# dattalab-6-cam/multicam-calibration

Hardware: AMD Instinct MI355X
Metric: LM iterations/sec (6 cams x 10k frames x 54 pts per GPU shard; + ms/Jacobian-eval) (higher is better)
Workload: dtype f64

## Files before the change

### multicam-calibration_amd/csrc/mcba_solve.hip

```cpp
#include <stdlib.h>
#include <algorithm>
#include "mcba_kernels.h"
#include "mcba_lm.h"
#include "mcba_math.h"
#include "mcba_backsub.h"

namespace mcba {

typedef double solve_d4 __attribute__((ext_vector_type(4)));

__device__ __forceinline__ double lane_bcast(double v, int lane) {
  union { double d; int i[2]; } a, b;
  a.d = v;
  b.i[0] = __builtin_amdgcn_readlane(a.i[0], lane);
  b.i[1] = __builtin_amdgcn_readlane(a.i[1], lane);
  return b.d;
}

__device__ __forceinline__ void wave_lds_sync() {
  __builtin_amdgcn_fence(__ATOMIC_RELEASE, "wavefront");
  __builtin_amdgcn_wave_barrier();
  __builtin_amdgcn_fence(__ATOMIC_ACQUIRE, "wavefront");
}

__device__ __forceinline__ double rsqrt_cubic(double a) {
  double y = __builtin_amdgcn_rsq(a);
  double e = fma(-a * y, y, 1.0);
  double q = e * fma(0.375, e, 0.5);
  return fma(y, q, y);
}

template <int NTHREADS>
__device__ __forceinline__ void block_reduce4(double (&v)[4], bool take_max, double* s_red) {
  const int wave = threadIdx.x >> 6, lane = threadIdx.x & 63;
#pragma unroll
  for (int off = 32; off >= 1; off >>= 1) {
#pragma unroll
    for (int c = 0; c < 4; ++c) {
      double o = __shfl_xor(v[c], off, 64);
      v[c] = take_max ? fmax(v[c], o) : v[c] + o;
    }
  }
  __syncthreads();
  if (lane == 0) {
#pragma unroll
    for (int c = 0; c < 4; ++c) s_red[c * 16 + wave] = v[c];
  }
  __syncthreads();
#pragma unroll
  for (int c = 0; c < 4; ++c) {
    double r = s_red[c * 16];
    for (int w = 1; w < NTHREADS / 64; ++w) r = take_max ? fmax(r, s_red[c * 16 + w]) : r + s_red[c * 16 + w];
    v[c] = r;
  }
}

__device__ __forceinline__ void post_state(const SolveArgs& a, const double* st, bool write_back, bool stepped = false) {
  const int tid = threadIdx.x;
  if (tid < MCBA_LMS - 1) {
    const double v = st[tid];
    if (write_back) a.lms[tid] = v;
    if (a.host_state) a.host_state[tid] = v;
  }
  if (!a.host_state && !a.flag) return;
  __threadfence_system();
  __syncthreads();
  if (tid == 0) {
    if (a.host_state) *reinterpret_cast<volatile double*>(a.host_state + MCBA_LMS - 1) = a.seq;
    if (a.flag) __hip_atomic_store(a.flag, 4.0 * a.seq + (stepped ? 2.0 : 3.0), __ATOMIC_RELEASE, __HIP_MEMORY_SCOPE_AGENT);
  }
}

#define STAMP(k) do { } while (0)

#ifndef MCBA_SOLVE_LOOKAHEAD
#define MCBA_SOLVE_LOOKAHEAD 1
#endif
__host__ __device__ inline bool solve_lookahead(int npad) { return MCBA_SOLVE_LOOKAHEAD && npad <= 96; }

#ifndef MCBA_RL_NB
#define MCBA_RL_NB 4
#endif
__device__ __forceinline__ void rl_lds_barrier() { asm volatile("s_waitcnt lgkmcnt(0)\n\ts_barrier" ::: "memory"); }
__device__ __forceinline__ size_t rl_tile(int I, int J) { return ((size_t)(I * (I + 1) / 2 + J)) << 8; }
typedef double solve_d2 __attribute__((ext_vector_type(2)));
__device__ __forceinline__ solve_d4 rl_tile_load(const double* t, int lane) {
  const solve_d2 lo = *reinterpret_cast<const solve_d2*>(t + 2 * lane), hi = *reinterpret_cast<const solve_d2*>(t + 128 + 2 * lane);
  return solve_d4{lo[0], lo[1], hi[0], hi[1]};
}
__device__ __forceinline__ void rl_tile_store(double* t, int lane, const solve_d4 v) {
  *reinterpret_cast<solve_d2*>(t + 2 * lane) = solve_d2{v[0], v[1]};
  *reinterpret_cast<solve_d2*>(t + 128 + 2 * lane) = solve_d2{v[2], v[3]};
}
__device__ __forceinline__ int rl_pi(int lane) { return ((lane & 3) << 2) | ((lane >> 2) & 3) | (lane & 48); }

__device__ __forceinline__ solve_d4 rl_system_load(const double* __restrict__ S0, int n, int I, int J, int lane) {
  const int row = 16 * I + (lane & 15), c0 = 16 * J + 4 * (lane >> 4);
  const bool in = row <= n && c0 < n;
  return *reinterpret_cast<const solve_d4*>(S0 + (in ? (size_t)row * n + c0 : 0));
}
__device__ __forceinline__ solve_d4 rl_system_fixup(solve_d4 v, const double* damp, const unsigned char* fixed, int n, int I, int J, int lane) {
  const int row = 16 * I + (lane & 15), c0 = 16 * J + 4 * (lane >> 4);
  const bool in = row <= n && c0 < n;
#pragma unroll
  for (int r = 0; r < 4; ++r) {
    const int c = c0 + r;
    double x = in ? v[r] : ((row == c) ? 1.0 : 0.0);
    if (in && row == c) x += damp[row];
    v[r] = x;
  }
  if (fixed) {
#pragma unroll
    for (int r = 0; r < 4; ++r) {
      const int c = c0 + r;
      const bool fr = row < n && fixed[min(row, n - 1)] != 0, fc = c < n && fixed[min(c, n - 1)] != 0;
      if (fr || fc) v[r] = (row == c) ? 1.0 : 0.0;
    }
  }
  return v;
}
__device__ __forceinline__ solve_d4 rl_tile_from_system(const double* __restrict__ S0, const double* damp, const unsigned char* fixed, int n, int I, int J, int lane) {
  return rl_system_fixup(rl_system_load(S0, n, I, J, lane), damp, fixed, n, I, J, lane);
}

__device__ __forceinline__ solve_d4 rl_update(solve_d4 c, const solve_d4 pj, const solve_d4 pi) {
#pragma unroll
  for (int s = 0; s < 4; ++s) c = __builtin_amdgcn_mfma_f64_16x16x4f64(-pj[s], pi[s], c, 0, 0, 0);
  return c;
}

__device__ __forceinline__ void rl_unflatten(int t, int& Ir, int& Jr) {
  Ir = (int)((sqrt(8.0 * t + 1.0) - 1.0) * 0.5);
  while ((Ir + 1) * (Ir + 2) / 2 <= t) ++Ir;
  while (Ir * (Ir + 1) / 2 > t) --Ir;
  Jr = t - Ir * (Ir + 1) / 2;
}

constexpr int kRlMaxStagers = 16;
__host__ __device__ inline int rl_stagers(int npad) { const int nblk = npad >> 4, moff = (nblk - 1) * (nblk - 2) / 2; return min(kRlMaxStagers, max(1, moff / 8)); }
__device__ __forceinline__ double* rl_stage_flags(const SolveArgs& a, int nblk) { return a.work + 2 * rl_tile(nblk, 0) + 256 * 8; }
__device__ __forceinline__ unsigned long long* rl_stage_claims(const SolveArgs& a, int nblk) { return reinterpret_cast<unsigned long long*>(rl_stage_flags(a, nblk) + kRlMaxStagers); }
__device__ __forceinline__ unsigned long long rl_stage_tag(const SolveArgs& a) { return (unsigned long long)fabs(a.stage_tag); }
struct RlNoGate { __device__ __forceinline__ bool operator()() const { return true; } };
template <class Gate = RlNoGate>
__device__ __forceinline__ void rl_stage_offdiag(const SolveArgs& a, int part, int nparts, int lane, int wave, Gate gate = Gate()) {
  const int n = a.n, nblk = a.npad >> 4, m = nblk - 2;
  if (m <= 0) { (void)gate(); return; }
  const int M = m * (m + 1) / 2;
  const int t_begin = (int)(((long long)M * part) / nparts), ntile = (int)(((long long)M * (part + 1)) / nparts) - t_begin;
  if (ntile <= 0) (void)gate();
  const double* __restrict__ S0 = a.red;
  double* T1 = a.work;
  int Ir, Jr;
  rl_unflatten(t_begin, Ir, Jr);
  for (int done = 0; done < ntile; done += 8) {
    solve_d4 v[8];
    double* dstp[8];
    int Is[8], Js[8];
#pragma unroll
    for (int j = 0; j < 8; ++j) {
      const bool ok = done + j < ntile;
      Is[j] = ok ? Ir + 2 : nblk - 1; Js[j] = ok ? Jr + 1 : nblk - 2;
      dstp[j] = ok ? T1 + rl_tile(Is[j], Js[j]) : a.work + 2 * rl_tile(nblk, 0) + 256 * wave;
      v[j] = rl_system_load(S0, n, Is[j], Js[j], lane);
      if (++Jr > Ir) { ++Ir; Jr = 0; }
    }
    if (done == 0 && !gate()) return;
#pragma unroll
    for (int j = 0; j < 8; ++j) rl_tile_store(dstp[j], lane, rl_system_fixup(v[j], nullptr, a.fixed, n, Is[j], Js[j], lane));
  }
}
__device__ __forceinline__ void rl_stager(const SolveArgs& a, int b, int ns) {
  if (a.stage_tag < 0.0) return;
  const int lane = threadIdx.x & 63, wave = __builtin_amdgcn_readfirstlane(threadIdx.x >> 6), nw = blockDim.x >> 6;
  extern __shared__ double smem[];
  volatile int* s_mine_p = reinterpret_cast<volatile int*>(smem);
#define s_mine (*s_mine_p)
  auto gate = [&]() -> bool {
    if (threadIdx.x == 0) {
      if (a.stage_tag != floor(a.stage_tag)) {
        const long long t0 = wall_clock64();
        while (wall_clock64() - t0 < 20000000LL) __builtin_amdgcn_s_sleep(64);
      }
      const unsigned long long tag2 = 2 * rl_stage_tag(a);
      const unsigned long long old = __hip_atomic_fetch_max(rl_stage_claims(a, a.npad >> 4) + b, tag2, __ATOMIC_RELAXED, __HIP_MEMORY_SCOPE_AGENT);
      s_mine = old < tag2 ? 1 : 0;
    }
    __syncthreads();
    return s_mine != 0;
  };
  rl_stage_offdiag(a, b * nw + wave, ns * nw, lane, wave & 7, gate);
  if (!s_mine) return;
#undef s_mine
  __threadfence();
  __syncthreads();
  if (threadIdx.x == 0) __hip_atomic_store(rl_stage_flags(a, a.npad >> 4) + b, a.stage_tag, __ATOMIC_RELEASE, __HIP_MEMORY_SCOPE_AGENT);
}

template <int NTHREADS>
__device__ __forceinline__ void solve_right_looking(const SolveArgs& a, const double* __restrict__ S0, const unsigned char* fixed, const double* damp, double* yv, double* dv, double* invd,
                                                    double* linv , double* Pop , double* dtile , double* znext , int* stage_miss , double* tstamp) {
  constexpr int NW = NTHREADS / 64, SL = 32 / NW;
  static_assert(NW == 8, "8 wavefronts: 256 VGPRs each");
  constexpr int NWK = NW - NW / 4;
  const int n = a.n, npad = a.npad, nblk = npad >> 4;
  const int tid = threadIdx.x, lane = tid & 63;
  const int wave = __builtin_amdgcn_readfirstlane(tid >> 6);
  const bool worker = (wave & 3) != 0;
  const int wk = wave - 1 - (wave >> 2);
  const int li = lane & 15, lg = lane >> 4, lpi = rl_pi(lane);
  double* T1 = a.work;
  double* T2 = a.work + rl_tile(nblk, 0);
  for (int j = tid; j < npad; j += NTHREADS) yv[j] = 0.0;
  solve_d4 Zp[SL];
#pragma unroll
  for (int sl = 0; sl < SL; ++sl) {
    const int I = wave + NW * sl;
    Zp[sl] = solve_d4{0.0, 0.0, 0.0, 0.0};
    if (I >= 1 && I < nblk) Zp[sl] = rl_tile_from_system(S0, damp, fixed, n, I, 0, lane);
    if (I == 1 && I < nblk) *reinterpret_cast<solve_d4*>(znext + 4 * lane) = Zp[sl];
  }
  if (wave == 0) {
    const solve_d4 v = rl_tile_from_system(S0, damp, fixed, n, 0, 0, lane);
#pragma unroll
    for (int r = 0; r < 4; ++r) dtile[li * 17 + 4 * lg + r] = v[r];
  }
  __syncthreads();
  for (int k = 0; k < nblk; ++k) {
    const int r0 = 16 * k;
    if (wave == 0) {
      double r[16];
#pragma unroll
      for (int c = 0; c < 16; ++c) r[c] = lane < 16 ? dtile[li * 17 + c] : ((lane < 32 && c == li) ? 1.0 : 0.0);
      double myinv = 1.0;
      const int jmax = r0 + 16 <= n ? 16 : n - r0;
#pragma unroll
      for (int j = 0; j < 16; ++j) {
        if (j < jmax) {
          double s0 = 0.0, s1 = 0.0;
#pragma unroll
          for (int qq = 0; qq < j; ++qq) {
            const double ljq = lane_bcast(r[qq], j);
            if (qq & 1) s1 = fma(r[qq], ljq, s1); else s0 = fma(r[qq], ljq, s0);
          }
          r[j] -= s0 + s1;
          const double pj = lane_bcast(r[j], j);
          const double inv = rsqrt_cubic(pj);
          r[j] *= inv;
          myinv = lane == j ? inv : myinv;
        }
      }
      if (lane < 16) {
        invd[r0 + lane] = myinv;
        if (r0 + lane == n) {
#pragma unroll
          for (int c = 0; c < 16; ++c) if (c < lane) yv[r0 + c] = r[c];
        }
      } else if (lane < 32) {
#pragma unroll
        for (int c = 0; c < 16; ++c) linv[(r0 + li) * 17 + c] = r[c];
      }
    } else {
    const int mleft = nblk - k - 1;
    const int nwk = k == 0 || mleft * (mleft + 1) / 2 >= 48 ? NWK + 1 : NWK;
    const int wq = worker ? wk : NWK;
    if (!worker && k > 0) {
      for (int I = k; I < nblk; ++I) {
        solve_d4 x;
#pragma unroll
        for (int r = 0; r < 4; ++r) x[r] = Pop[256 * I + 4 * ((4 * lg + r) + 16 * (li >> 2)) + (li & 3)];
        *reinterpret_cast<solve_d4*>(T2 + rl_tile(I, k - 1) + 64 * lg + 4 * li) = x;
      }
    }
    if (wq >= nwk) {
    } else if (k == 0) {
      {
        solve_d4 v[4];
        int Id[4];
#pragma unroll
        for (int j = 0; j < 4; ++j) {
          Id[j] = 1 + wq + nwk * j;
          v[j] = rl_system_load(S0, n, min(Id[j], nblk - 1), min(Id[j], nblk - 1), lane);
        }
#pragma unroll
        for (int j = 0; j < 4; ++j) {
          if (Id[j] < nblk) rl_tile_store(T1 + rl_tile(Id[j], Id[j]), lane, rl_system_fixup(v[j], damp, fixed, n, Id[j], Id[j], lane));
        }
        for (int Ix = 1 + wq + nwk * 4; Ix < nblk; Ix += nwk)
          rl_tile_store(T1 + rl_tile(Ix, Ix), lane, rl_tile_from_system(S0, damp, fixed, n, Ix, Ix, lane));
      }
      if (wave == 1) {
        const int ns = (int)gridDim.x - 1;
        const double* fl = rl_stage_flags(a, nblk);
        const int lb = min(lane, kRlMaxStagers - 1);
        bool ok = lane >= ns;
        for (int polls = 0; polls < 40000 && !__all(ok); ++polls) {
          if (!ok) ok = __hip_atomic_load(fl + lb, __ATOMIC_RELAXED, __HIP_MEMORY_SCOPE_AGENT) == fabs(a.stage_tag);
          if (!__all(ok)) __builtin_amdgcn_s_sleep(8);
        }
        bool abandoned = false;
        if (!ok) {
          const unsigned long long tag2 = 2 * rl_stage_tag(a);
          const unsigned long long old = __hip_atomic_fetch_max(rl_stage_claims(a, nblk) + lb, tag2 + 1, __ATOMIC_RELAXED, __HIP_MEMORY_SCOPE_AGENT);
          if (old == tag2) {
            while (__hip_atomic_load(fl + lb, __ATOMIC_RELAXED, __HIP_MEMORY_SCOPE_AGENT) != fabs(a.stage_tag)) __builtin_amdgcn_s_sleep(8);
          } else {
            abandoned = true;
          }
        }
        const unsigned long long gone = __ballot(abandoned);
        __builtin_amdgcn_fence(__ATOMIC_ACQUIRE, "agent");
        if (lane == 0) *stage_miss = (int)(gone & 0xFFFFu);
      }
    } else if (k + 1 < nblk) {
      const int J0 = k + 1, m = nblk - J0;
      const int M = m * (m + 1) / 2;
      const int t_begin = (int)(((long long)M * wq) / nwk), ntile = (int)(((long long)M * (wq + 1)) / nwk) - t_begin;
      if (ntile > 0) {
        constexpr int R = MCBA_RL_NB;
        double* const dummy = a.work + 2 * rl_tile(nblk, 0) + 256 * wave;
        int Ir, Jr, issued = 0;
        rl_unflatten(t_begin, Ir, Jr);
        solve_d4 cin[R];
        int It[R], Jt[R];
        double* dst[R];
        auto request = [&](int j) {
          const bool ok = issued < ntile;
          It[j] = ok ? Ir + J0 : nblk - 1; Jt[j] = ok ? Jr + J0 : nblk - 1;
          double* tp = T1 + rl_tile(It[j], Jt[j]);
          dst[j] = ok ? tp : dummy;
          cin[j] = rl_tile_load(tp, lane);
          ++issued;
          if (++Jr > Ir) { ++Ir; Jr = 0; }
        };
#pragma unroll
        for (int j = 0; j < R; ++j) request(j);
        solve_d4 pi_n = *reinterpret_cast<const solve_d4*>(Pop + 256 * It[0] + 4 * lane);
        solve_d4 pj_n = *reinterpret_cast<const solve_d4*>(Pop + 256 * Jt[0] + 4 * lpi);
        for (int done = 0; done < ntile; done += R) {
#pragma unroll
          for (int j = 0; j < R; ++j) {
            const solve_d4 pi = pi_n, pj = pj_n;
            const int jn = (j + 1) % R;
            pi_n = *reinterpret_cast<const solve_d4*>(Pop + 256 * It[jn] + 4 * lane);
            pj_n = *reinterpret_cast<const solve_d4*>(Pop + 256 * Jt[jn] + 4 * lpi);
            const solve_d4 out = rl_update(cin[j], pj, pi);
            rl_tile_store(dst[j], lane, out);
            request(j);
          }
        }
      }
    }
    }
    __syncthreads();
    if (k == 0 && ((int)gridDim.x == 1 || *stage_miss)) {
      const int ns = (int)gridDim.x - 1, gone = ns == 0 ? 1 : *stage_miss, nsh = ns == 0 ? 1 : ns;
      for (int b = 0; b < nsh; ++b)
        if ((gone >> b) & 1) rl_stage_offdiag(a, b * NW + wave, nsh * NW, lane, wave);
      __syncthreads();
    }
    {
      solve_d4 cpre[SL];
#pragma unroll
      for (int sl = 0; sl < SL; ++sl) {
        const int I = wave + NW * sl;
        cpre[sl] = solve_d4{0.0, 0.0, 0.0, 0.0};
        if (I >= k + 1 && I < nblk) cpre[sl] = rl_tile_load(T1 + rl_tile(I, k + 1), lane);
      }
      solve_d4 lv;
#pragma unroll
      for (int s2 = 0; s2 < 4; ++s2) lv[s2] = linv[(r0 + 4 * lg + s2) * 17 + (lpi & 15)];
      solve_d4 pja = {0.0, 0.0, 0.0, 0.0};
      if (k + 1 < nblk) {
        const solve_d4 zn = *reinterpret_cast<const solve_d4*>(znext + 256 * (k & 1) + 4 * lpi);
#pragma unroll
        for (int s2 = 0; s2 < 4; ++s2) pja = __builtin_amdgcn_mfma_f64_16x16x4f64(lv[s2], zn[s2], pja, 0, 0, 0);
      }
#pragma unroll
      for (int sl = 0; sl < SL; ++sl) {
        const int I = wave + NW * sl;
        if (I > k && I < nblk) {
          solve_d4 xo = {0.0, 0.0, 0.0, 0.0};
#pragma unroll
          for (int s2 = 0; s2 < 4; ++s2) xo = __builtin_amdgcn_mfma_f64_16x16x4f64(lv[s2], Zp[sl][s2], xo, 0, 0, 0);
          *reinterpret_cast<solve_d4*>(Pop + 256 * I + 4 * lane) = xo;
          if (16 * I + li == n) {
#pragma unroll
            for (int r = 0; r < 4; ++r) yv[r0 + 4 * lg + r] = xo[r];
          }
          const solve_d4 c = rl_update(cpre[sl], pja, xo);
          if (I == k + 1) {
#pragma unroll
            for (int r = 0; r < 4; ++r) dtile[li * 17 + 4 * lg + r] = c[r];
          } else {
            Zp[sl] = c;
            if (I == k + 2) *reinterpret_cast<solve_d4*>(znext + 256 * ((k + 1) & 1) + 4 * lane) = c;
          }
        }
      }
    }
    __syncthreads();
  }
  {
    solve_d4 wc[4], wn[4];
    auto fetch = [&](int kk, solve_d4 (&w)[4]) {
      const bool ok = kk >= 1 && tid < 16 * kk;
      const double* src = T2 + rl_tile(ok ? kk : 1, ok ? (tid >> 4) : 0) + 4 * (tid & 15);
#pragma unroll
      for (int q = 0; q < 4; ++q) w[q] = *reinterpret_cast<const solve_d4*>(src + 64 * q);
    };
    auto step = [&](int k, solve_d4 (&w)[4], solve_d4 (&wnext)[4]) {
      const int r0 = 16 * k;
      fetch(k - 1, wnext);
      if (tid < 16) {
        const double* lr = linv + (r0 + tid) * 17;
        double s4[4] = {0.0, 0.0, 0.0, 0.0};
#pragma unroll
        for (int c = 0; c < 16; ++c) s4[c & 3] = fma(lr[c], yv[r0 + c], s4[c & 3]);
        dv[r0 + tid] = (r0 + tid < n) ? (s4[0] + s4[1]) + (s4[2] + s4[3]) : 0.0;
      }
      rl_lds_barrier();
      if (tid < r0) {
        double s0 = yv[tid], s1 = 0.0;
#pragma unroll
        for (int q = 0; q < 4; ++q) {
          s0 = fma(-w[q][0], dv[r0 + 4 * q], s0);
          s1 = fma(-w[q][1], dv[r0 + 4 * q + 1], s1);
          s0 = fma(-w[q][2], dv[r0 + 4 * q + 2], s0);
          s1 = fma(-w[q][3], dv[r0 + 4 * q + 3], s1);
        }
        yv[tid] = s0 + s1;
      }
      rl_lds_barrier();
    };
    fetch(nblk - 1, wc);
    for (int k = nblk - 1; k >= 0; k -= 2) {
      step(k, wc, wn);
      if (k >= 1) step(k - 1, wn, wc);
    }
  }
}

constexpr int kStageMax = 7;

template <int NTHREADS, bool LDSW, int KS>
__device__ __forceinline__ void solve_cam_body(const SolveArgs& a) {
  constexpr int kStage = KS;
  extern __shared__ double smem[];
  const int n = a.n, npad = a.npad, nblk = npad >> 4;
  const int tid = threadIdx.x, wave = tid >> 6, lane = tid & 63;
  constexpr int NW = NTHREADS / 64;
  constexpr int RS = NTHREADS / 16;
  double* panel = smem;
  double* yv = panel + (size_t)npad * 17;
  double* dv = yv + npad;
  double* invd = dv + npad;
  double* damp = invd + npad;
  double* s_red = damp + npad;
  int* s_flag = reinterpret_cast<int*>(s_red + 64);
  double* lst = s_red + 72;
  double* W = lst + MCBA_LMS;
  const int ldw = npad + 1;
  double* linv = W + (size_t)npad * ldw;
  double* pnext = linv + (size_t)nblk * 16 * 17;
  constexpr int kLookWave = 2;
  const bool lookahead = LDSW && NW == 4 && solve_lookahead(npad);
  double* Bs = lst + MCBA_LMS;
  const int bst = npad + 2;

  const double* __restrict__ S0 = a.red;
  const double* __restrict__ diagU = a.red + (size_t)n * n + n;
  const double* __restrict__ gc = diagU + n;
  const double* __restrict__ scal = gc + n;
  const unsigned char* fixed = a.fixed;
  const int rr = tid >> 4, cc = tid & 15;

  double stage[LDSW ? kStage * kStage : 1];
  if (LDSW) {
#pragma unroll
    for (int ia = 0; ia < kStage; ++ia) {
      const int i = rr + RS * ia;
#pragma unroll
      for (int b = 0; b < kStage; ++b) {
        const int j = cc + 16 * b;
        const bool need = i <= n && j < n && j <= i;
        stage[ia * kStage + b] = S0[need ? i * n + j : 0];
      }
    }
  }

  if (tid < MCBA_LMS) lst[tid] = a.lms_in[tid];
  double gm = 0.0;
  for (int i = tid; i < npad; i += NTHREADS) {
    const bool in = i < n, fx = in && fixed && fixed[i];
    const double dsc = (in && a.dscale) ? a.dscale[a.cw == 12 ? i : 12 * (i / 6) + 6 + i % 6] : 0.0;
    const double du = in ? (dsc > 0.0 ? dsc : diagU[i]) : 1.0;
    damp[i] = du > 0.0 ? du : 1.0;
    if (in && !fx) gm = fmax(gm, fabs(gc[i]));
  }
  if (tid < 12) gm = fmax(gm, scal[4 + tid]);
  const double frame_fail = scal[2];
  double red4[4] = {gm, 0.0, 0.0, 0.0};
  block_reduce4<NTHREADS>(red4, true, s_red);
  const double g_inf = red4[0];
  double* lms = lst;
  if (lms[MCBA_LM_DONE] != 0.0) {
    post_state(a, lst, false);
    return;
  }
  if (tid == 0) {
    int mode = 0;
    lms[MCBA_LM_TICK] += 1.0;
    if (a.decide) {
      if (lms[MCBA_LM_SKIP] != 0.0) lm_mark_rebuild(lms);
      else if (a.red[(size_t)n * n + 3 * n + 16 + 5] != 0.0) {
        lm_mark_rebuild(lms);
        lms[MCBA_LM_SKIP] = 1.0;
        lms[MCBA_LM_SOLVE_INFO] = 4.0;
        mode = 3;
      } else {
        const double lam_spec = lm_spec_lambda(lms[1], a.lam_min, a.dec_floor);
        lm_decide(a.red + (size_t)n * n + 3 * n + 16, DecideArgs{2, 0.0, 0.0, 0.0, a.lam_min, a.lam_max, lms, a.ftol, a.xtol, a.dec_floor});
        if (!(lms[4] != 0.0 && lms[1] == lam_spec)) {
          lms[MCBA_LM_SKIP] = 1.0;
          lms[MCBA_LM_SOLVE_INFO] = 3.0;
          mode = 3;
        }
      }
    }
    if (mode == 0) {
      lms[MCBA_LM_GINF] = g_inf;
      const double pending = lms[MCBA_LM_PENDING];
      if (pending != 0.0) { lms[MCBA_LM_DONE] = pending; mode = 1; }
      else if (g_inf < a.gtol) { lms[MCBA_LM_DONE] = 1.0; mode = 1; }
      else if (frame_fail != 0.0) mode = 2;
    }
    s_flag[0] = mode;
  }
  __syncthreads();
  const int mode = s_flag[0];
  if (mode == 1 || mode == 3) {
    post_state(a, lst, true);
    return;
  }
  STAMP(0);
  const double lambda = lms[1];
  const int sel = static_cast<int>(lms[3]) & 1;
  const double* xc = sel ? a.x1 : a.x0;

  if (mode == 0) {
    for (int i = tid; i < npad; i += NTHREADS) damp[i] *= lambda;
    __syncthreads();
    if constexpr (!LDSW) {
      static_assert(NTHREADS == 512, "the right-looking variant is written for 8 wavefronts");
      STAMP(1);
      solve_right_looking<NTHREADS>(a, S0, fixed, damp, yv, dv, invd, panel, Bs, Bs + (size_t)16 * bst, Bs + (size_t)16 * bst + 16 * 17, s_flag + 2, lst);
    } else {
    {
#pragma unroll
      for (int ia = 0; ia < kStage; ++ia) {
        const int i = rr + RS * ia;
#pragma unroll
        for (int b = 0; b < kStage; ++b) {
          const int j = cc + 16 * b;
          if (i <= n && j < n && j <= i) W[i * ldw + j] = stage[ia * kStage + b] + ((i == j) ? damp[i] : 0.0);
        }
      }
    }
    for (int e = n * npad + n + tid; e < npad * npad; e += NTHREADS) {
      const int i = e / npad, j = e - i * npad;
      if (j <= i && (i > n || j == n)) W[(size_t)i * ldw + j] = (i == j) ? 1.0 : 0.0;
    }
    __syncthreads();
    if (fixed) {
      for (int e = tid; e < (n + 1) * npad; e += NTHREADS) {
        const int i = e / npad, j = e - i * npad;
        if (j < n && j <= i && ((i < n && fixed[i]) || fixed[j])) W[(size_t)i * ldw + j] = (i == j) ? 1.0 : 0.0;
      }
      __syncthreads();
    }
    const int q = lane < 16 ? lane : 16 + 48 * wave + (lane - 16);
    STAMP(1);
#define LAP(i) do { } while (0)
    for (int k = 0; k < nblk; ++k) {
      const int r0 = 16 * k, ntile = nblk - k;
      if (k > 0) {
        {
          const int p_lo = lookahead ? r0 - 16 : 0;
          for (int t = wave; t < ntile; t += NW) {
            const int R = r0 + 16 * t;
            solve_d4 acc = {0.0, 0.0, 0.0, 0.0};
            if (lookahead && k > 1) {
#pragma unroll
              for (int reg = 0; reg < 4; ++reg) acc[reg] = pnext[(16 * t + 4 * reg + (lane >> 4)) * 17 + (lane & 15)];
            }
            const double* pa = W + (size_t)(R + (lane & 15)) * ldw + (lane >> 4);
            const double* pb = W + (size_t)(r0 + (lane & 15)) * ldw + (lane >> 4);
            for (int p = p_lo; p < r0; p += 16) {
              double av[4], bv[4];
#pragma unroll
              for (int u = 0; u < 4; ++u) { av[u] = pa[p + 4 * u]; bv[u] = pb[p + 4 * u]; }
#pragma unroll
              for (int u = 0; u < 4; ++u) acc = __builtin_amdgcn_mfma_f64_16x16x4f64(av[u], bv[u], acc, 0, 0, 0);
            }
#pragma unroll
            for (int reg = 0; reg < 4; ++reg) panel[(16 * t + 4 * reg + (lane >> 4)) * 17 + (lane & 15)] = acc[reg];
          }
        }
        __syncthreads();
      }
      LAP(0);
      const bool idrow = LDSW && wave == NW - 1 && lane >= 48;
      if (lookahead && wave == kLookWave && k >= 1 && k + 1 < nblk) {
        const int r1 = r0 + 16;
        const double* pb = W + (size_t)(r1 + (lane & 15)) * ldw + (lane >> 4);
        for (int t = 0; t < ntile - 1; ++t) {
          solve_d4 acc = {0.0, 0.0, 0.0, 0.0};
          const double* pa = W + (size_t)(r1 + 16 * t + (lane & 15)) * ldw + (lane >> 4);
          for (int p = 0; p < r0; p += 16) {
            double av[4], bv[4];
#pragma unroll
            for (int u = 0; u < 4; ++u) { av[u] = pa[p + 4 * u]; bv[u] = pb[p + 4 * u]; }
#pragma unroll
            for (int u = 0; u < 4; ++u) acc = __builtin_amdgcn_mfma_f64_16x16x4f64(av[u], bv[u], acc, 0, 0, 0);
          }
#pragma unroll
          for (int reg = 0; reg < 4; ++reg) pnext[(16 * t + 4 * reg + (lane >> 4)) * 17 + (lane & 15)] = acc[reg];
        }
      }
      if (wave == 0 || 16 + 48 * wave < 16 * ntile || (LDSW && wave == NW - 1)) {
        const bool rv = q < 16 * ntile;
        double r[16];
        {
          const double* wsrc = W + (size_t)(r0 + (rv ? q : 0)) * ldw + r0;
#pragma unroll
          for (int c = 0; c < 16; ++c) r[c] = wsrc[c];
          if (k > 0) {
#pragma unroll
            for (int c = 0; c < 16; ++c) r[c] -= panel[(rv ? q : 0) * 17 + c];
          }
          if (idrow) {
#pragma unroll
            for (int c = 0; c < 16; ++c) r[c] = (c == lane - 48) ? 1.0 : 0.0;
          }
        }
        double myinv = 1.0;
        const int jmax = r0 + 16 <= n ? 16 : n - r0;
#pragma unroll
        for (int j = 0; j < 16; ++j) {
          if (j < jmax) {
            double s0 = 0.0, s1 = 0.0;
#pragma unroll
            for (int qq = 0; qq < j; ++qq) {
              const double ljq = lane_bcast(r[qq], j);
              if (qq & 1) s1 = fma(r[qq], ljq, s1); else s0 = fma(r[qq], ljq, s0);
            }
            r[j] -= s0 + s1;
            const double pj = lane_bcast(r[j], j);
            const double inv = rsqrt_cubic(pj);
            r[j] *= inv;
            myinv = lane == j ? inv : myinv;
          }
        }
        if (rv && (lane >= 16 || wave == 0)) {
          double* wr = W + (size_t)(r0 + q) * ldw + r0;
#pragma unroll
          for (int c = 0; c < 16; ++c) wr[c] = r[c];
        }
        if (wave == 0 && lane < 16) invd[r0 + lane] = myinv;
        if (idrow) {
          double* li = linv + (k * 16 + (lane - 48)) * 17;
#pragma unroll
          for (int c = 0; c < 16; ++c) li[c] = r[c];
        }
      }
      __syncthreads();
      LAP(1);
    }

    STAMP(2);
    if (wave == 0) {
      static_assert(16 * KS <= 128, "two columns per lane cover the LDS-resident systems");
      const int j0 = lane, j1 = lane + 64, jc0 = min(j0, npad - 1);
      double y0 = j0 < n ? W[(size_t)n * ldw + j0] : 0.0, y1 = j1 < n ? W[(size_t)n * ldw + j1] : 0.0;
      if (j0 < npad) yv[j0] = y0;
      if (j1 < npad) yv[j1] = y1;
      double wn[16];
#pragma unroll
      for (int t = 0; t < 16; ++t) wn[t] = W[(size_t)(16 * (nblk - 1) + t) * ldw + jc0];
      wave_lds_sync();
#pragma unroll
      for (int k = KS - 1; k >= 0; --k) {
        if (k < nblk) {
          const int r0 = 16 * k;
          double wc[16];
#pragma unroll
          for (int t = 0; t < 16; ++t) wc[t] = wn[t];
          const double* li = linv + (k * 16 + (lane & 15)) * 17;
          double s[4] = {0.0, 0.0, 0.0, 0.0};
#pragma unroll
          for (int c = 0; c < 16; ++c) s[c & 3] = fma(li[c], yv[r0 + c], s[c & 3]);
          if (k > 0) {
#pragma unroll
            for (int t = 0; t < 16; ++t) wn[t] = W[(size_t)(r0 - 16 + t) * ldw + jc0];
          }
          const double dk = (r0 + (lane & 15) < n) ? (s[0] + s[1]) + (s[2] + s[3]) : 0.0;
          if (lane < 16) {
            dv[r0 + lane] = dk;
            if (r0 + lane < n) a.dc[r0 + lane] = dk;
          }
          wave_lds_sync();
          if (j0 < r0) {
            double s0 = y0, s1 = 0.0;
#pragma unroll
            for (int t = 0; t < 16; t += 2) { s0 = fma(-wc[t], dv[r0 + t], s0); s1 = fma(-wc[t + 1], dv[r0 + t + 1], s1); }
            y0 = s0 + s1;
            yv[j0] = y0;
          }
          if (k > 4 && j1 < r0) {
            const double* wp = W + (size_t)r0 * ldw + j1;
            double s0 = y1, s1 = 0.0;
#pragma unroll
            for (int t = 0; t < 16; t += 2) { s0 = fma(-wp[(size_t)t * ldw], dv[r0 + t], s0); s1 = fma(-wp[(size_t)(t + 1) * ldw], dv[r0 + t + 1], s1); }
            y1 = s0 + s1;
            yv[j1] = y1;
          }
          wave_lds_sync();
        }
      }
    }
    __syncthreads();
    if (a.flag && tid == 0) __hip_atomic_store(a.flag, 4.0 * a.seq + 1.0, __ATOMIC_RELEASE, __HIP_MEMORY_SCOPE_AGENT);
    }
  }

  STAMP(3);
  double sums[4] = {0.0, 0.0, 0.0, 0.0};
  if (mode == 0) {
    for (int i = tid; i < n; i += NTHREADS) {
      const double d = dv[i], xv = xc[a.cw == 12 ? i : 12 * (i / 6) + 6 + i % 6];
      if constexpr (!LDSW) a.dc[i] = d;
      sums[3] += (fabs(d) < 1e300) ? 0.0 : 1.0;
      sums[0] += d * (damp[i] * d - gc[i]);
      sums[1] += d * d;
      sums[2] += xv * xv;
    }
  }
  if constexpr (!LDSW) {
    if (a.flag && mode == 0) {
      __threadfence();
      __syncthreads();
      if (tid == 0) __hip_atomic_store(a.flag, 4.0 * a.seq + 1.0, __ATOMIC_RELEASE, __HIP_MEMORY_SCOPE_AGENT);
    }
  }
  block_reduce4<NTHREADS>(sums, false, s_red);
  if (tid == 0) {
    const bool failed = mode == 2 || sums[3] != 0.0 || !(fabs(sums[0]) < 1e300);
    lms[MCBA_LM_SOLVE_INFO] = mode == 2 ? 2.0 : failed ? 1.0 : 0.0;
    if (failed) {
      const double lam = fmin(lambda * lms[2], a.lam_max);
      lms[1] = lam;
      lms[2] *= 2.0;
      lms[MCBA_LM_SKIP] = 1.0;
      if (lam >= a.lam_max) lms[MCBA_LM_DONE] = 3.0;
    } else {
      lms[MCBA_LM_SKIP] = 0.0;
      lms[MCBA_LM_PRED_CAM] = sums[0];
      lms[MCBA_LM_DCN2] = sums[1];
      lms[MCBA_LM_XCN2] = sums[2];
    }
  }
  __syncthreads();
  post_state(a, lst, true, a.flag != nullptr && mode == 0 && lms[MCBA_LM_DONE] == 0.0 && lms[MCBA_LM_SKIP] == 0.0);
}

template <int NTHREADS, bool LDSW, int KS>
__global__ __launch_bounds__(NTHREADS) void k_solve_cam(SolveArgs a) {
  if constexpr (!LDSW) {
    if (blockIdx.x > 0) { rl_stager(a, (int)blockIdx.x - 1, (int)gridDim.x - 1); return; }
  }
  solve_cam_body<NTHREADS, LDSW, KS>(a);
}

struct BacksubArgs {
  Sel sl;
  const double *rec0, *rec1, *fbuf;
  double *x0, *x1, *bpart;
  int C, F, Fpad;
  BacksubWait wait;
};
template <int KS, int CW = 12>
__global__ __launch_bounds__(64 * kBacksubWaves) void k_solve_backsub(SolveArgs a, BacksubArgs b) {
  __shared__ double s_t[kBacksubWaves][6][64];
  __shared__ double s_mail[8 + 12 * 9];
  if (blockIdx.x == 0) {
    if (threadIdx.x < 256) solve_cam_body<256, true, KS>(a);
    return;
  }
  b.wait.mail = s_mail;
  backsub_body<DevStep, CW>(b.sl, b.rec0, b.rec1, b.fbuf, DevStep{a.dc}, b.x0, b.x1, b.bpart, b.C, b.F, b.Fpad, (int)blockIdx.x - 1, b.C < kBacksubWaves ? b.C : kBacksubWaves, s_t, &b.wait);
}

size_t solve_lds_bytes(int npad, int use_lds) {
  size_t d = (size_t)npad * 17 + 4 * (size_t)npad + 72 + MCBA_LMS;
  d += use_lds ? (size_t)npad * (npad + 1) + (size_t)(npad / 16) * 16 * 17 + (solve_lookahead(npad) ? (size_t)npad * 17 : 0) : (size_t)16 * (npad + 2) + 16 * 17 + 2 * 256;
  return d * sizeof(double);
}

int solve_fits_lds(int npad, int lds_limit) { return npad <= 16 * kStageMax && solve_lds_bytes(npad, 1) <= (size_t)lds_limit - 10 * 1024; }

static const void* solve_kernel(int npad, int use_lds) {
  if (use_lds) return npad <= 80 ? reinterpret_cast<const void*>(&k_solve_cam<256, true, 5>) : reinterpret_cast<const void*>(&k_solve_cam<256, true, kStageMax>);
  return reinterpret_cast<const void*>(&k_solve_cam<512, false, 1>);
}

int solve_set_lds_limit(int npad, int use_lds) {
  size_t bytes = solve_lds_bytes(npad, use_lds);
  if (bytes <= 64 * 1024) return 0;
  return hipFuncSetAttribute(solve_kernel(npad, use_lds), hipFuncAttributeMaxDynamicSharedMemorySize, (int)bytes) == hipSuccess ? 0 : 1;
}

int solve_backsub_set_lds_limit(int npad, int cw) {
  const size_t bytes = solve_lds_bytes(npad, 1) + sizeof(double) * (kBacksubWaves * 6 * 64 + 8 + 12 * 9);
  if (bytes <= 64 * 1024) return 0;
  const void* k = cw == 6 ? (npad <= 80 ? reinterpret_cast<const void*>(&k_solve_backsub<5, 6>) : reinterpret_cast<const void*>(&k_solve_backsub<kStageMax, 6>))
                          : (npad <= 80 ? reinterpret_cast<const void*>(&k_solve_backsub<5>) : reinterpret_cast<const void*>(&k_solve_backsub<kStageMax>));
  return hipFuncSetAttribute(k, hipFuncAttributeMaxDynamicSharedMemorySize, (int)solve_lds_bytes(npad, 1)) == hipSuccess ? 0 : 1;
}

void launch_solve_backsub(hipStream_t st, const SolveArgs& a, Sel sl, const double* rec0, const double* rec1, const double* fbuf, double* x0, double* x1, double* bpart, int C, int F, int Fpad,
                          const double* early_state, int max_polls, int spec, double* timeout_dev, double* timeout_host, int strict) {
  BacksubArgs b{sl, rec0, rec1, fbuf, x0, x1, bpart, C, F, Fpad, BacksubWait{early_state, a.flag, a.dc, nullptr, a.seq, max_polls, spec, a.lam_min, timeout_dev, timeout_host, a.dec_floor, strict}};
  const size_t lds = solve_lds_bytes(a.npad, 1);
  const dim3 grid(1 + Fpad / 64), block(64 * kBacksubWaves);
  if (a.cw == 6) {
    if (a.npad <= 80) hipLaunchKernelGGL((k_solve_backsub<5, 6>), grid, block, lds, st, a, b);
    else hipLaunchKernelGGL((k_solve_backsub<kStageMax, 6>), grid, block, lds, st, a, b);
  } else if (a.npad <= 80) hipLaunchKernelGGL((k_solve_backsub<5>), grid, block, lds, st, a, b);
  else hipLaunchKernelGGL((k_solve_backsub<kStageMax>), grid, block, lds, st, a, b);
}

void launch_solve_cam(hipStream_t st, const SolveArgs& a) {
  size_t lds = solve_lds_bytes(a.npad, a.use_lds);
  if (a.use_lds) {
    if (a.npad <= 80) hipLaunchKernelGGL((k_solve_cam<256, true, 5>), dim3(1), dim3(256), lds, st, a);
    else hipLaunchKernelGGL((k_solve_cam<256, true, kStageMax>), dim3(1), dim3(256), lds, st, a);
    return;
  }
  int ns = rl_stagers(a.npad);
  SolveArgs b = a;
  if (const char* e = getenv("MCBA_SOLVE_STAGERS")) {
    const int v = atoi(e);
    if (v == -2) b.stage_tag += 0.5;
    else if (v < 0) b.stage_tag = -b.stage_tag;
    else ns = std::min(kRlMaxStagers, v);
  }
  hipLaunchKernelGGL((k_solve_cam<512, false, 1>), dim3(1 + ns), dim3(512), lds, st, b);
}

}
```

Baseline: 9907.

## Shorten camera-solve prologue and epilogue with per-wave reductions and early flag release

Restructures the camera block solve's setup and finish. The gradient max-norm now uses a single-wave reduction instead of a block reduction plus barrier. In the non-decide path the lambda-scaled diagonal is staged into LDS before the mode decision, and the damping rows and x-norm loads are done in registers. The final step reductions run on one or two wavefronts, and the completion flag is released before the host-state fence. The aim is to cut block-wide barriers and serial latency per LM iteration, at the cost of more complex control flow and a hard-coded assumption of at most 128 unknowns.

```diff
diff --git a/multicam-calibration_amd/csrc/mcba_solve.hip b/multicam-calibration_amd/csrc/mcba_solve.hip
--- a/multicam-calibration_amd/csrc/mcba_solve.hip
+++ b/multicam-calibration_amd/csrc/mcba_solve.hip
@@ -55,20 +55,27 @@
   }
 }
 
-__device__ __forceinline__ void post_state(const SolveArgs& a, const double* st, bool write_back, bool stepped = false) {
+
+__device__ __forceinline__ double mul_rounded(double x, double y) {
+#pragma clang fp contract(off)
+  return x * y;
+}
+
+__device__ __forceinline__ void release_final(const SolveArgs& a, bool stepped) {
+  if (a.flag) __hip_atomic_store(a.flag, 4.0 * a.seq + (stepped ? 2.0 : 3.0), __ATOMIC_RELEASE, __HIP_MEMORY_SCOPE_AGENT);
+}
+
+__device__ __forceinline__ void post_state(const SolveArgs& a, const double* st, bool write_back) {
   const int tid = threadIdx.x;
   if (tid < MCBA_LMS - 1) {
     const double v = st[tid];
     if (write_back) a.lms[tid] = v;
     if (a.host_state) a.host_state[tid] = v;
   }
-  if (!a.host_state && !a.flag) return;
+  if (!a.host_state) return;
   __threadfence_system();
   __syncthreads();
-  if (tid == 0) {
-    if (a.host_state) *reinterpret_cast<volatile double*>(a.host_state + MCBA_LMS - 1) = a.seq;
-    if (a.flag) __hip_atomic_store(a.flag, 4.0 * a.seq + (stepped ? 2.0 : 3.0), __ATOMIC_RELEASE, __HIP_MEMORY_SCOPE_AGENT);
-  }
+  if (tid == 0) *reinterpret_cast<volatile double*>(a.host_state + MCBA_LMS - 1) = a.seq;
 }
 
 #define STAMP(k) do { } while (0)
@@ -484,34 +491,102 @@
       for (int b = 0; b < kStage; ++b) {
         const int j = cc + 16 * b;
         const bool need = i <= n && j < n && j <= i;
-        stage[ia * kStage + b] = S0[need ? i * n + j : 0];
-      }
-    }
-  }
-
-  if (tid < MCBA_LMS) lst[tid] = a.lms_in[tid];
-  double gm = 0.0;
-  for (int i = tid; i < npad; i += NTHREADS) {
-    const bool in = i < n, fx = in && fixed && fixed[i];
-    const double dsc = (in && a.dscale) ? a.dscale[a.cw == 12 ? i : 12 * (i / 6) + 6 + i % 6] : 0.0;
-    const double du = in ? (dsc > 0.0 ? dsc : diagU[i]) : 1.0;
-    damp[i] = du > 0.0 ? du : 1.0;
-    if (in && !fx) gm = fmax(gm, fabs(gc[i]));
-  }
-  if (tid < 12) gm = fmax(gm, scal[4 + tid]);
+        stage[ia * kStage + b] = S0[need ? (unsigned)(i * n + j) : 0u];
+      }
+    }
+  }
+
+  const auto xrow = [&](int i) { return a.cw == 12 ? i : 12 * (i / 6) + 6 + i % 6; };
+  const double st_mine = a.lms_in[tid < MCBA_LMS ? tid : 0];
+  const double st_done = a.lms_in[MCBA_LM_DONE], st_pending = a.lms_in[MCBA_LM_PENDING], st_lambda = a.lms_in[1], st_sel = a.lms_in[3], st_tick = a.lms_in[MCBA_LM_TICK];
   const double frame_fail = scal[2];
-  double red4[4] = {gm, 0.0, 0.0, 0.0};
-  block_reduce4<NTHREADS>(red4, true, s_red);
-  const double g_inf = red4[0];
+  constexpr int GR = LDSW ? (16 * KS + 63) / 64 : 8;
+  double gv[GR];
+  unsigned char gfix[GR];
+#pragma unroll
+  for (int g = 0; g < GR; ++g) { gv[g] = gc[min(lane + 64 * g, n - 1)]; gfix[g] = 0; }
+  if (fixed) {
+#pragma unroll
+    for (int g = 0; g < GR; ++g) gfix[g] = fixed[min(lane + 64 * g, n - 1)];
+  }
+  const double gs = scal[4 + min(lane, 11)];
+  const auto damp_of = [&](int i, double du, double dsc) {
+    const double d = i < n ? (dsc > 0.0 ? dsc : du) : 1.0;
+    return d > 0.0 ? d : 1.0;
+  };
+  constexpr int ND = LDSW ? kStage : 1;
+  double dd[ND], dsc[ND];
+  if constexpr (LDSW) {
+    static_assert(RS == 16, "the diagonal of the staged triangle lies with the threads rr == cc");
+#pragma unroll
+    for (int ia = 0; ia < ND; ++ia) { dd[ia] = diagU[min(rr + RS * ia, n - 1)]; dsc[ia] = 0.0; }
+    if (a.dscale) {
+#pragma unroll
+      for (int ia = 0; ia < ND; ++ia) dsc[ia] = a.dscale[xrow(min(rr + RS * ia, n - 1))];
+    }
+  } else {
+    for (int i = tid; i < npad; i += NTHREADS) {
+      const int ic = min(i, n - 1);
+      const double d = damp_of(i, diagU[ic], a.dscale ? a.dscale[xrow(ic)] : 0.0);
+      damp[i] = a.decide ? d : mul_rounded(st_lambda, d);
+    }
+  }
+  constexpr int kXcWave = 2;
+  double xq0[2] = {0.0, 0.0}, xq1[2] = {0.0, 0.0};
+  if (LDSW && wave == kXcWave) {
+#pragma unroll
+    for (int g = 0; g < 2; ++g) { const int xi = xrow(min(lane + 64 * g, n - 1)); xq0[g] = a.x0[xi]; xq1[g] = a.x1[xi]; }
+  }
+  if constexpr (LDSW) {
+    if (tid == 0) W[(size_t)n * ldw + n] = 1.0;
+    for (int i = n + 1 + rr; i < npad; i += RS) {
+      for (int j = cc; j <= i; j += 16) W[(size_t)i * ldw + j] = (i == j) ? 1.0 : 0.0;
+    }
+  }
+  if (tid < MCBA_LMS) lst[tid] = st_mine;
   double* lms = lst;
-  if (lms[MCBA_LM_DONE] != 0.0) {
+  if (st_done != 0.0) {
+    if (tid == 0) release_final(a, false);
     post_state(a, lst, false);
     return;
   }
-  if (tid == 0) {
-    int mode = 0;
-    lms[MCBA_LM_TICK] += 1.0;
-    if (a.decide) {
+  const auto stage_to_lds = [&](double lam) {
+    if constexpr (LDSW) {
+#pragma unroll
+      for (int ia = 0; ia < kStage; ++ia) {
+        const int i = rr + RS * ia;
+        const double ld = mul_rounded(lam, damp_of(i, dd[ia], dsc[ia]));
+        if (rr == cc && i < n) damp[i] = ld;
+#pragma unroll
+        for (int b = 0; b < kStage; ++b) {
+          const int j = cc + 16 * b;
+          if (i <= n && j < n && j <= i) W[i * ldw + j] = stage[ia * kStage + b] + ((i == j) ? ld : 0.0);
+        }
+      }
+    }
+  };
+  if (!a.decide) stage_to_lds(st_lambda);
+  double gm = 0.0;
+#pragma unroll
+  for (int g = 0; g < GR; ++g) {
+    if (lane + 64 * g < n && !gfix[g]) gm = fmax(gm, fabs(gv[g]));
+  }
+  if (lane < 12) gm = fmax(gm, gs);
+  const double g_inf = wave_max(gm);
+  wave_lds_sync();
+  int mode = 0;
+  double lambda = st_lambda, selw = st_sel;
+  if (!a.decide) {
+    if (st_pending != 0.0 || g_inf < a.gtol) mode = 1;
+    else if (frame_fail != 0.0) mode = 2;
+    if (tid == 0) {
+      lms[MCBA_LM_TICK] = st_tick + 1.0;
+      lms[MCBA_LM_GINF] = g_inf;
+      if (mode == 1) lms[MCBA_LM_DONE] = st_pending != 0.0 ? st_pending : 1.0;
+    }
+  } else {
+    if (tid == 0) {
+      lms[MCBA_LM_TICK] += 1.0;
       if (lms[MCBA_LM_SKIP] != 0.0) lm_mark_rebuild(lms);
       else if (a.red[(size_t)n * n + 3 * n + 16 + 5] != 0.0) {
         lm_mark_rebuild(lms);
@@ -527,51 +602,46 @@
           mode = 3;
         }
       }
-    }
-    if (mode == 0) {
-      lms[MCBA_LM_GINF] = g_inf;
-      const double pending = lms[MCBA_LM_PENDING];
-      if (pending != 0.0) { lms[MCBA_LM_DONE] = pending; mode = 1; }
-      else if (g_inf < a.gtol) { lms[MCBA_LM_DONE] = 1.0; mode = 1; }
-      else if (frame_fail != 0.0) mode = 2;
-    }
-    s_flag[0] = mode;
-  }
-  __syncthreads();
-  const int mode = s_flag[0];
+      if (mode == 0) {
+        lms[MCBA_LM_GINF] = g_inf;
+        const double pending = lms[MCBA_LM_PENDING];
+        if (pending != 0.0) { lms[MCBA_LM_DONE] = pending; mode = 1; }
+        else if (g_inf < a.gtol) { lms[MCBA_LM_DONE] = 1.0; mode = 1; }
+        else if (frame_fail != 0.0) mode = 2;
+      }
+      s_flag[0] = mode;
+    }
+    __syncthreads();
+    mode = s_flag[0];
+    lambda = lms[1];
+    selw = lms[3];
+    if constexpr (!LDSW) {
+      for (int i = tid; i < npad; i += NTHREADS) damp[i] = mul_rounded(lambda, damp[i]);
+    }
+  }
   if (mode == 1 || mode == 3) {
+    if (tid == 0) release_final(a, false);
+    __syncthreads();
     post_state(a, lst, true);
     return;
   }
   STAMP(0);
-  const double lambda = lms[1];
-  const int sel = static_cast<int>(lms[3]) & 1;
-  const double* xc = sel ? a.x1 : a.x0;
+  const int sel = static_cast<int>(selw) & 1;
 
   if (mode == 0) {
-    for (int i = tid; i < npad; i += NTHREADS) damp[i] *= lambda;
-    __syncthreads();
     if constexpr (!LDSW) {
       static_assert(NTHREADS == 512, "the right-looking variant is written for 8 wavefronts");
+      __syncthreads();
       STAMP(1);
       solve_right_looking<NTHREADS>(a, S0, fixed, damp, yv, dv, invd, panel, Bs, Bs + (size_t)16 * bst, Bs + (size_t)16 * bst + 16 * 17, s_flag + 2, lst);
     } else {
-    {
-#pragma unroll
-      for (int ia = 0; ia < kStage; ++ia) {
-        const int i = rr + RS * ia;
-#pragma unroll
-        for (int b = 0; b < kStage; ++b) {
-          const int j = cc + 16 * b;
-          if (i <= n && j < n && j <= i) W[i * ldw + j] = stage[ia * kStage + b] + ((i == j) ? damp[i] : 0.0);
-        }
-      }
-    }
-    for (int e = n * npad + n + tid; e < npad * npad; e += NTHREADS) {
-      const int i = e / npad, j = e - i * npad;
-      if (j <= i && (i > n || j == n)) W[(size_t)i * ldw + j] = (i == j) ? 1.0 : 0.0;
-    }
+    if (a.decide) stage_to_lds(lambda);
     __syncthreads();
+    if (wave == kXcWave) {
+      const double s0 = wave_sum(lane < n ? 0.0 + (sel ? xq1[0] : xq0[0]) * (sel ? xq1[0] : xq0[0]) : 0.0);
+      const double s1 = wave_sum(lane + 64 < n ? 0.0 + (sel ? xq1[1] : xq0[1]) * (sel ? xq1[1] : xq0[1]) : 0.0);
+      if (lane == 0) s_red[0] = s0 + s1;
+    }
     if (fixed) {
       for (int e = tid; e < (n + 1) * npad; e += NTHREADS) {
         const int i = e / npad, j = e - i * npad;
@@ -736,24 +806,42 @@
 
   STAMP(3);
   double sums[4] = {0.0, 0.0, 0.0, 0.0};
-  if (mode == 0) {
-    for (int i = tid; i < n; i += NTHREADS) {
-      const double d = dv[i], xv = xc[a.cw == 12 ? i : 12 * (i / 6) + 6 + i % 6];
-      if constexpr (!LDSW) a.dc[i] = d;
-      sums[3] += (fabs(d) < 1e300) ? 0.0 : 1.0;
-      sums[0] += d * (damp[i] * d - gc[i]);
-      sums[1] += d * d;
-      sums[2] += xv * xv;
-    }
-  }
-  if constexpr (!LDSW) {
+  if constexpr (LDSW) {
+    if (mode == 0 && wave == 0) {
+      double pr[2], d2[2];
+      unsigned long long bad = 0;
+#pragma unroll
+      for (int g = 0; g < 2; ++g) {
+        const int i = lane + 64 * g, ic = min(i, n - 1);
+        const double d = dv[ic], dm = damp[ic], gi = gc[ic];
+        pr[g] = i < n ? 0.0 + d * (dm * d - gi) : 0.0;
+        d2[g] = i < n ? 0.0 + d * d : 0.0;
+        bad |= __ballot(i < n && !(fabs(d) < 1e300));
+      }
+      sums[0] = wave_sum(pr[0]) + wave_sum(pr[1]);
+      sums[1] = wave_sum(d2[0]) + wave_sum(d2[1]);
+      sums[2] = s_red[0];
+      sums[3] = bad != 0 ? 1.0 : 0.0;
+    }
+  } else {
+    const double* xc = sel ? a.x1 : a.x0;
+    if (mode == 0) {
+      for (int i = tid; i < n; i += NTHREADS) {
+        const double d = dv[i], xv = xc[xrow(i)];
+        a.dc[i] = d;
+        sums[3] += (fabs(d) < 1e300) ? 0.0 : 1.0;
+        sums[0] += d * (damp[i] * d - gc[i]);
+        sums[1] += d * d;
+        sums[2] += xv * xv;
+      }
+    }
     if (a.flag && mode == 0) {
       __threadfence();
       __syncthreads();
       if (tid == 0) __hip_atomic_store(a.flag, 4.0 * a.seq + 1.0, __ATOMIC_RELEASE, __HIP_MEMORY_SCOPE_AGENT);
     }
-  }
-  block_reduce4<NTHREADS>(sums, false, s_red);
+    block_reduce4<NTHREADS>(sums, false, s_red);
+  }
   if (tid == 0) {
     const bool failed = mode == 2 || sums[3] != 0.0 || !(fabs(sums[0]) < 1e300);
     lms[MCBA_LM_SOLVE_INFO] = mode == 2 ? 2.0 : failed ? 1.0 : 0.0;
@@ -769,9 +857,10 @@
       lms[MCBA_LM_DCN2] = sums[1];
       lms[MCBA_LM_XCN2] = sums[2];
     }
+    release_final(a, mode == 0 && lms[MCBA_LM_DONE] == 0.0 && lms[MCBA_LM_SKIP] == 0.0);
   }
   __syncthreads();
-  post_state(a, lst, true, a.flag != nullptr && mode == 0 && lms[MCBA_LM_DONE] == 0.0 && lms[MCBA_LM_SKIP] == 0.0);
+  post_state(a, lst, true);
 }
 
 template <int NTHREADS, bool LDSW, int KS>
```

Result: no change. 10000, median of 6 (+0.9%).
